# SixLabors/ZlibStream

Measured on AMD Instinct MI355X. Metric: deflate MB/s (input) at level 6, 64 MiB buffers, higher is better.
Workload: dtype u8; 1 GPU; english64: 1 x 67108864-byte pseudo-random-English (Zipf words of alice29.txt) buffer per GPU, level 6, zlib framing, inputs resident in HBM; level=6, buffer_bytes=67108864, buffers_per_gpu=1, compressed_bytes=27425826, parallelism=independent buffers, 1 GPU(s), no collective in the data path

## Files before the change

### zlibstream_amd/csrc/zs_core.h

```cpp
#pragma once
#include <stdint.h>
#include <vector>

#if defined(__HIPCC__)
#include <hip/hip_runtime.h>
#define ZS_HD __host__ __device__ __forceinline__
#define ZS_HD_NOINLINE __host__ __device__
#else
#define ZS_HD inline
#define ZS_HD_NOINLINE
#endif

namespace zs {

constexpr int kMinMatch = 3;
constexpr int kMaxMatch = 258;
constexpr int kMinLookahead = kMaxMatch + kMinMatch + 1;
constexpr int kWSize = 32768;
constexpr int kWMask = kWSize - 1;
constexpr int kWindowSize = 2 * kWSize;
constexpr int kMaxDist = kWSize - kMinLookahead;
constexpr int kSlideAt = kWindowSize - kMinLookahead;
constexpr int kHashBits = 15;
constexpr int kHashSize = 1 << kHashBits;
// ... 479 lines not shown
        uint32_t cK = acc.mK(p), cK4 = acc.mK4(p);
        if (p == 0) cK = cK4 = kNoMatch;
        const Step st = lazy_step(kind, p, pend, cK, cK4, lv);
        if (st.emit) ns++;
        kind = st.kind;
        p = st.pos;
    }
    int node = node_of3(kind, p, cx.cs, ce);
    while (node < kNodeExit3) {
        const uint32_t v = tbl[node];
        ns += node_cnt(v);
        node = node_succ(v);
    }
    return (uint32_t)(node - kNodeExit3) | flags | ((uint32_t)ns << 16);
}

ZS_HD bool slot_valid(const ChunkCtx &cx, int slot, int64_t body_end) {
    if (slot <= 256) return cx.cs + slot <= body_end + 257;
    return cx.cs > 0;
}


ZS_HD int extra_lbits(int code) { return code < 8 ? 0 : (code == 28 ? 0 : (code - 4) >> 2); }
ZS_HD int extra_dbits(int code) { return code < 4 ? 0 : (code - 2) >> 1; }
ZS_HD int extra_blbits(int code) { return code == 16 ? 2 : code == 17 ? 3 : code == 18 ? 7 : 0; }
ZS_HD int base_length(int code) {
    if (code < 8) return code;
    if (code == 28) return 0;
    int e = (code - 4) >> 2;
    return ((4 + (code & 3)) << e);
// ... 507 lines not shown
```

### zlibstream_amd/csrc/zs_device.h

```cpp
#pragma once
#include <cstddef>
#include "zs_core.h"
#include "zs_lit_engine.h"
#include "zs_fast_sweep.h"
#include "zs_rle.h"

namespace zs {

constexpr int kMatchTile = 16384;
constexpr int kMatchBack = 32512;
constexpr int kMatchFwd = 272;
constexpr int kMatchLdsBytes = kMatchBack + kMatchTile + kMatchFwd;
constexpr int kMatchLdsLinks = kMatchBack + kMatchTile;
constexpr int kMatchLds = kMatchLdsBytes + 2 * kMatchLdsLinks;
constexpr int kAdlerPiece = 65536;

constexpr int64_t kScratchWindow = 0;
constexpr int64_t kScratchHead = 66560;
constexpr int64_t kScratchPrev = kScratchHead + 2 * kHashSize;
constexpr int64_t kScratchHead32 = kScratchPrev + 2 * kWSize;
constexpr int64_t kScratchBytes = kScratchHead32 + 4 * kHashSize;

struct StreamDesc {
    const uint8_t *in;
// ... 94 lines not shown
constexpr uint32_t kSpecBail = 1u << 30;
ZS_HD uint32_t spec_pack(int guess, int exit_slot, int count, bool bail) {
    return (uint32_t)guess | ((uint32_t)exit_slot << 9) | ((uint32_t)count << 18) | (bail ? kSpecBail : 0u);
}
ZS_HD int spec_guess(uint32_t r) { return (int)(r & 0x1FF); }
ZS_HD int spec_exit(uint32_t r) { return (int)((r >> 9) & 0x1FF); }
ZS_HD int spec_count(uint32_t r) { return (int)((r >> 18) & 0xFFF); }
constexpr int kSpecMinInput = 1 << 20;
constexpr int kSpecLenBits = 10;
constexpr int kSpecWarm = 128;
constexpr int kSpecRunsDen = 8;
struct K5Spec {
    uint32_t *rec;
    uint32_t *base;
    int len_bits, warm, corrupt;
};
constexpr int kDeferBudget = 8;
constexpr int kCutBudget = 12;

constexpr int kFastChunk = 262144;
constexpr int kFastWarm = 65536;
constexpr int kFastMinInput = 4 << 20;
constexpr int kFastMinPeriodic = 64 << 10;
constexpr int64_t kFastRunSyms = kFastWarm + kFastChunk + 1024;
constexpr int64_t kFastRunBitWords = (kFastWarm + kFastChunk + 2048) / 32;
constexpr int64_t kFastRunScratch = 2 * kHashSize + 4 * kHashSize;
struct FastRunOut {
    int64_t mark_pos, mark_nsyms;
    int64_t end_pos, nsyms;
    int64_t final_base;
    int64_t sym_dst;
// ... 13 lines not shown
```

### zlibstream_amd/csrc/zs_engine.hip

```cpp
#include <hip/hip_runtime.h>

#include <algorithm>
#include <cstdio>
#include <cstdlib>
#include <cstring>
#include <string>
#include <thread>
#include <vector>

#define ZS_BUILDING_LIBRARY
#include "../../include/zsgpu.h"
#include "zs_kernels.hip"
#include "zs_inflate_par.hip"
#include "zs_inflate_tok.hip"
#include "zs_png.hip"
#include "zs_crc32.hip"

using namespace zs;

namespace {

struct DevBuf {
    void *p = nullptr;
    size_t cap = 0;
};

enum Stage {
    kStClear, kStAdler, kStLinks, kStMatch, kStChunkMap, kStSegMap, kStResolve, kStExpand, kStEmitSyms, kStTail, kStTrees,
    kStOffsets, kStEmitBits, kStSpecWalk, kStSpecVerify, kStCrc32, kStCount
};
const char *const kStageNames[kStCount] = {"clear", "adler", "links", "match", "chunkmap", "segmap", "resolve", "expand",
                                           "emit_syms", "tail", "trees", "offsets", "emit_bits", "spec_walk", "spec_verify", "crc32_frame"};

}

struct zs_ctx {
    int device = 0;
    hipStream_t stream = nullptr;
    hipStream_t aux = nullptr;
    hipEvent_t ev_fork = nullptr, ev_join = nullptr, ev_pre0 = nullptr, ev_pre = nullptr;
    hipEvent_t ev_spec[2] = {};
    hipEvent_t ev_part[16] = {};
    std::vector<hipEvent_t> ev_pool;
    std::string err;
    bool profiling = false;
    int fast_fallbacks = 0;
    int round_runs = 0;
    int cut_rounds = 0;
    int lit_fallbacks = 0;
    int spec_streams = 0, spec_fallbacks = 0, spec_wrong_chunks = 0;
    int spec_periodic = 0;
    int64_t dbg_blk_off = 0, dbg_chunk_off = 0, dbg_nchunks = 0, dbg_spec_n = 0, dbg_n_spec = 0;
    int64_t lit_engine_bytes = 0;
    std::vector<int64_t> inf_used;
    int64_t *inf_probe = nullptr;
    int64_t png_segments = 0;
    int fast_rounds = 0;
    bool no_rounds_once = false;
    int last_op = 0;
    hipEvent_t ev[kStCount + 1] = {};
    double stage_ms[kStCount] = {};
    uint32_t *crc_tab = nullptr;
    DevBuf sd, st, work, wpre, geo, link, mm, maps, chunk_far, segmap, supmap, seg_entry, seg_symbase, seg_stale, entry, symbase, stale, syms, blk_end, blk_top, blocks, trees, info, pieces, scratch,
        stage_in, stage_out, wr, inf_desc, inf_state, par_ps, par_st, par_work, par_cbits, par_ccnt, par_surv, par_scnt, par_cands, par_tabs, par_toktabs, par_toks, par_ctoks, par_tokstat, par_tails, par_retry, par_fxtab, par_blocks, par_cells,
        par_windows, par_fail, run_syms, run_bits, run_scratch, run_outs, run_fail, adl_tr, adl_res, plan_blk, ins_bits, mm_bak, cut_pos, cut_bkt, win_groups, win_sg, win_maps, win_entries, persist_bak, resume_flag, rle_tiles, own_in, fr_chunks, fr_meta, fr_planes, fr_prov, fr_base, fr_counters, spec_rec, spec_flags, png_img, png_seg, png_ctr, png_fimg, png_scratch, png_a7img, png_inflated, png_passes, crc_desc, crc_res, png_zs, png_gather;
    uint32_t *crc32_tab = nullptr;
    hipEvent_t ev_crc[2] = {};
    bool resume_poisoned = false;
    void *pinned = nullptr;
    size_t pinned_cap = 0;
    void *pin_io = nullptr;
    size_t pin_io_cap = 0;
    bool pin_io_busy = false;
    void *pin_out = nullptr;
    size_t pin_out_cap = 0;
    bool pin_out_busy = false;
};

namespace {

// ... 419 lines not shown
    size_t n_work = pl.w_clear.size() + pl.w_adler.size() + pl.w_links.size() + pl.w_match.size() + pl.w_chunks.size() +
                    pl.w_segs.size() + pl.w_sups.size() + pl.w_blocks.size() + pl.w_runs.size();
    if (!ensure(c, c->sd, sizeof(StreamDesc) * (size_t)n) || !ensure(c, c->st, sizeof(StreamState) * (size_t)n) ||
        !ensure(c, c->work, sizeof(uint2) * (n_work + 1)) || !ensure(c, c->link, 2 * (size_t)pl.n_pos + 64) ||
        !ensure(c, c->mm, 8 * (size_t)pl.n_pos + 256) ||
        !ensure(c, c->maps, 4 * (size_t)(pl.n_chunks + 1) * kSlots) || !ensure(c, c->segmap, 8 * (size_t)(pl.n_segs + 1) * kSlots) ||
        !ensure(c, c->supmap, 8 * (size_t)(pl.n_sups + 1) * kSlots) || !ensure(c, c->chunk_far, 2 * (size_t)pl.n_chunks + 64) ||
        !ensure(c, c->seg_entry, 2 * (size_t)(pl.n_segs + 2)) || !ensure(c, c->seg_symbase, 4 * (size_t)(pl.n_segs + 2)) ||
        !ensure(c, c->seg_stale, (size_t)pl.n_segs + 64) || !ensure(c, c->entry, 2 * (size_t)(pl.n_chunks + 2)) ||
        !ensure(c, c->symbase, 4 * (size_t)(pl.n_chunks + 2)) || !ensure(c, c->stale, (size_t)pl.n_chunks + 64) ||
        !ensure(c, c->syms, 4 * (size_t)pl.n_syms + 64) || !ensure(c, c->blk_end, 4 * (size_t)pl.n_blocks + 64) ||
        !ensure(c, c->blk_top, 4 * (size_t)pl.n_blocks + 64) || !ensure(c, c->blocks, sizeof(BlockRec) * (size_t)pl.n_blocks) ||
        !ensure(c, c->trees, sizeof(TreeWork) * (size_t)pl.n_blocks) || !ensure(c, c->info, sizeof(BlockInfo) * (size_t)pl.n_blocks) ||
        !ensure(c, c->pieces, 4 * (size_t)pl.n_pieces + 64) || !ensure(c, c->scratch, (size_t)kScratchBytes * (size_t)n) ||
        !ensure(c, c->cut_pos, 8 * (size_t)pl.n_cuts + 64) || !ensure(c, c->cut_bkt, 8 * (size_t)pl.n_cuts + 64) ||
        (pl.n_spec && (!ensure(c, c->spec_rec, 8 * (size_t)pl.n_spec + 64) || !ensure(c, c->spec_flags, 4 * (size_t)n + 64))))
        return false;
    const size_t o_segcl = 16 * (size_t)pl.n_segs, o_cstart = o_segcl + 4 * ((size_t)pl.n_segs + (size_t)n),
                 o_head = o_cstart + 4 * ((size_t)pl.n_chunks + (size_t)n), o_cl = o_head + 4 * (size_t)pl.n_chunks;
    const size_t geo_bytes = o_cl + 4 * pl.cl.size();
    if (!ensure(c, c->geo, geo_bytes + 64)) return false;
    for (int i = 0; i < n; i++) {
        StreamDesc &s = pl.sd[(size_t)i];
        const int32_t *g = (const int32_t *)c->geo.p;
        const uint8_t *gb = (const uint8_t *)c->geo.p;
        s.seg_c0 = g + s.seg_off, s.seg_after = g + pl.n_segs + s.seg_off, s.seg_base = g + 2 * pl.n_segs + s.seg_off;
        s.seg_S = g + 3 * pl.n_segs + s.seg_off;
        s.seg_cl = (const int32_t *)(gb + o_segcl) + s.seg_off + i;
        s.cstart = (const int32_t *)(gb + o_cstart) + s.chunk_off + i;
        s.head = (const int32_t *)(gb + o_head) + s.chunk_off;
        s.cl = (const uint32_t *)(gb + o_cl);
// ... 104 lines not shown
        hipLaunchKernelGGL(zs_zero_kernel, dim3(blocks), dim3(256), 0, stream, z);
        if (ro && ro->resume && pl.sd[0].fv_end >= 0) {
            const int64_t lo = std::max<int64_t>(0, ro->p0 - kWSize - 64) / 32, hi = ro->p0 / 32;
            if (hi > lo) ZS_HIP(c, hipMemsetAsync(pl.sd[0].ins_bits + lo, 0xFF, (size_t)(hi - lo) * 4, stream));
            ZS_HIP(c, hipMemsetD32Async((hipDeviceptr_t)(pl.sd[0].ins_bits + hi), (int)((1u << (ro->p0 & 31)) - 1u), 1, stream));
        }
    }

    const StreamDesc *d_sd = dev<StreamDesc>(c->sd);
    StreamState *d_st = dev<StreamState>(c->st);
    const uint2 *d_work = dev<uint2>(c->work);
    const bool prof = c->profiling;
    const int k5_ahead = getenv("ZS_K5_AHEAD") ? atoi(getenv("ZS_K5_AHEAD")) : 1;
    c->dbg_blk_off = pl.sd[0].blk_off, c->dbg_chunk_off = pl.sd[0].chunk_off, c->dbg_nchunks = pl.sd[0].nchunks;
    c->dbg_spec_n = pl.sd[0].spec_n, c->dbg_n_spec = pl.n_spec;
    const K5Spec k5s{dev<uint32_t>(c->spec_rec), dev<uint32_t>(c->spec_rec) + pl.n_spec, spec_bits, spec_warm, spec_corrupt};
    int spec_ok_streams = 0;
    bool need_maps = true, spec_ran = false;
    if (!rounds) c->spec_streams = c->spec_fallbacks = c->spec_wrong_chunks = c->spec_periodic = 0;
    auto mark = [&](int i) {
        if (prof) (void)hipEventRecord(c->ev[i], stream);
    };
    ht_plan = ht_us();
    ZS_HIP(c, hipEventRecord(c->ev_pre0, stream));
    auto side_work = [&]() -> bool {
        ZS_HIP(c, hipStreamWaitEvent(c->aux, c->ev_pre0, 0));
        if (!pl.w_clear.empty())
            hipLaunchKernelGGL(zs_clear_kernel, dim3((unsigned)pl.w_clear.size()), dim3(256), 0, c->aux, d_sd, d_work + o_clear);
        if (!pl.w_adler.empty())
            hipLaunchKernelGGL(zs_adler_kernel, dim3((unsigned)pl.w_adler.size()), dim3(256), 0, c->aux, d_sd, d_work + o_adler,
                               dev<uint32_t>(c->pieces));
// ... 218 lines not shown
        ZS_HIP(c, hipMemcpyAsync(c->sd.p, c->pinned, sizeof(StreamDesc) * (size_t)n, hipMemcpyHostToDevice, stream));
        if (getenv("ZS_DEBUG")) fprintf(stderr, "zs: %d stream(s) below 4 MiB at level %d: %s\n", n, level, periodic ? "all period, the speculative runs" : "the sweeps");
    }
    mark(3);
    if (strategy == kHuffmanOnly) {
        ZS_HIP(c, hipMemsetAsync(c->mm.p, 0, 8 * (size_t)pl.n_pos + 64, stream));
    } else if (!pl.w_match.empty())
        hipLaunchKernelGGL(zs_match_kernel, dim3((unsigned)pl.w_match.size()), dim3(1024), kMatchLds + 16, stream, d_sd, d_work + o_match,
                           dev<uint16_t>(c->link), dev<uint2>(c->mm), lv, strategy, d_st);
    mark(4);
    if (!side_work()) return false;
    if (pl.n_spec) {
        spec_ran = true;
        hipLaunchKernelGGL((zs_emit_syms_lane_kernel<4, 1>), dim3((unsigned)((pl.max_spec_n + 63) / 64), (unsigned)n), dim3(kK5Threads), 0, stream, d_sd, d_st,
                           (const uint2 *)nullptr, 0, dev<uint2>(c->mm), dev<uint16_t>(c->link), (const uint16_t *)nullptr, (const uint32_t *)nullptr,
                           dev<uint32_t>(c->syms), dev<int32_t>(c->blk_end), dev<int32_t>(c->blk_top), c->crc_tab, lv, strategy, hash_variant, k5_ahead, k5s);
        if (prof) (void)hipEventRecord(c->ev_spec[0], stream);
        hipLaunchKernelGGL(zs_spec_verify_kernel, dim3((unsigned)n), dim3(1024), 0, stream, d_sd, d_st, dev<uint2>(c->mm), dev<uint16_t>(c->link), c->crc_tab, lv,
                           strategy, hash_variant, k5s, dev<int32_t>(c->spec_flags));
        int32_t *hf = (int32_t *)c->pinned;
        ZS_HIP(c, hipMemcpyAsync(hf, c->spec_flags.p, 4 * (size_t)n, hipMemcpyDeviceToHost, stream));
        ZS_HIP(c, hipStreamSynchronize(stream));
        if (prof) (void)hipEventRecord(c->ev_spec[1], stream);
        for (int i = 0; i < n; i++) {
            if (hf[i] == 0) continue;
            c->spec_streams++;
            if (hf[i] == 1) spec_ok_streams++;
            else c->spec_fallbacks++;
            if (hf[i] == 2) c->spec_periodic++;
        }
        if (spec_ok_streams < c->spec_streams) {
// ... 122 lines not shown
                           dev<uint8_t>(c->scratch), c->crc_tab, lv, strategy, hash_variant, level);
        ZS_HIP(c, hipEventRecord(c->ev_join, c->aux));
    }
    if (!pl.w_segs.empty() && need_maps)
        hipLaunchKernelGGL(zs_expand_kernel, dim3((unsigned)((pl.w_segs.size() + 63) / 64)), dim3(64), 0, stream, d_sd, d_st,
                           d_work + o_segs, (int)pl.w_segs.size(), dev<uint2>(c->mm), dev<uint16_t>(c->link),
                           dev<uint32_t>(c->maps), dev<uint16_t>(c->seg_entry), dev<uint32_t>(c->seg_symbase),
                           dev<uint8_t>(c->stale), dev<uint16_t>(c->entry), dev<uint32_t>(c->symbase), c->crc_tab, lv, strategy,
                           hash_variant);
    mark(8);
    if (!pl.w_chunks.empty() && need_maps)
        hipLaunchKernelGGL((zs_emit_syms_lane_kernel<4, 0>), dim3((unsigned)((pl.w_chunks.size() + 63) / 64)), dim3(kK5Threads), 0, stream, d_sd, d_st,
                           d_work + o_chunks, (int)pl.w_chunks.size(), dev<uint2>(c->mm), dev<uint16_t>(c->link), dev<uint16_t>(c->entry),
                           dev<uint32_t>(c->symbase), dev<uint32_t>(c->syms), dev<int32_t>(c->blk_end), dev<int32_t>(c->blk_top),
                           c->crc_tab, lv, strategy, hash_variant, k5_ahead, k5s);
    if (spec_ok_streams)
        hipLaunchKernelGGL((zs_emit_syms_lane_kernel<4, 2>), dim3((unsigned)((pl.max_spec_n + 63) / 64), (unsigned)n), dim3(kK5Threads), 0, stream, d_sd, d_st,
                           (const uint2 *)nullptr, 0, dev<uint2>(c->mm), dev<uint16_t>(c->link), (const uint16_t *)nullptr, (const uint32_t *)nullptr,
                           dev<uint32_t>(c->syms), dev<int32_t>(c->blk_end), dev<int32_t>(c->blk_top), c->crc_tab, lv, strategy, hash_variant, k5_ahead, k5s);
    mark(9);
    if (tail_serial)
        hipLaunchKernelGGL(zs_tail_kernel, dim3((unsigned)n), dim3(1024), kTailLds, stream, d_sd, d_st, dev<uint16_t>(c->link),
                           dev<uint32_t>(c->syms), dev<int32_t>(c->blk_end), dev<int32_t>(c->blk_top), dev<BlockRec>(c->blocks),
                           dev<uint8_t>(c->scratch), c->crc_tab, lv, strategy, hash_variant, level);
    else if (!tail_late) ZS_HIP(c, hipStreamWaitEvent(stream, c->ev_join, 0));
    hipLaunchKernelGGL(zs_body_blocks_kernel, dim3((unsigned)n), dim3(256), 0, stream, d_sd, d_st, dev<int32_t>(c->blk_end),
                       dev<int32_t>(c->blk_top), dev<BlockRec>(c->blocks), dev<uint32_t>(c->syms));
    if (tail_late)
        hipLaunchKernelGGL(zs_tail_kernel, dim3((unsigned)n), dim3(1024), kTailLds, stream, d_sd, d_st, dev<uint16_t>(c->link),
                           dev<uint32_t>(c->syms), dev<int32_t>(c->blk_end), dev<int32_t>(c->blk_top), dev<BlockRec>(c->blocks),
                           dev<uint8_t>(c->scratch), c->crc_tab, lv, strategy, hash_variant, level);
    }
    if (pl.n_runs) {
        if (!getenv("ZS_FAST_NO_PROBE") && force_seq == 0 && !pl.any_dual) {
// ... 104 lines not shown
        for (size_t k = 0; k < nw && k < 24; k++) fprintf(stderr, " %d(end %lld, flush %d)", wb[k], (long long)wr->ends[k], wr->flush.empty() ? 0 : wr->flush[k]);
        fprintf(stderr, "\n");
    }
    if (prof) {
        for (int i = 0; i < kStCount; i++) {
            float ms = 0;
            if (i >= kStLinks && i <= kStEmitBits) (void)hipEventElapsedTime(&ms, c->ev[i], c->ev[i + 1]);
            c->stage_ms[i] = ms;
        }
        if (spec_ran) {
            float a = 0, b = 0, m = 0;
            (void)hipEventElapsedTime(&a, c->ev[kStChunkMap], c->ev_spec[0]);
            (void)hipEventElapsedTime(&b, c->ev_spec[0], c->ev_spec[1]);
            (void)hipEventElapsedTime(&m, c->ev_spec[1], c->ev[kStChunkMap + 1]);
            c->stage_ms[kStSpecWalk] = a, c->stage_ms[kStSpecVerify] = b, c->stage_ms[kStChunkMap] = m;
        }
        if (n_parts) {
            for (int i = kStLinks; i <= kStTail; i++) c->stage_ms[i] = 0;
            for (const TimedPair &t : pairs) {
                float ms = 0;
                (void)hipEventElapsedTime(&ms, t.a, t.b);
                c->stage_ms[t.stage] += ms;
            }
        }
    }
    {
        bool any_poison = false;
        std::vector<uint8_t> fl(force_lit ? *force_lit : std::vector<uint8_t>((size_t)n, 0));
        for (int i = 0; i < n; i++)
            if (hst[i].poison) any_poison = true, fl[(size_t)i] = 1;
// ... 184 lines not shown
    if (hipFuncGetAttributes(&fa, (const void *)zs_match_kernel) != hipSuccess || fa.sharedSizeBytes != 0) {
        fprintf(stderr, "zsgpu: zs_match_kernel has static LDS; its tile addressing assumes none\n");
        zs_ctx_destroy(c);
        return ZS_STREAM_ERROR;
    }
    *out = c;
    return ZS_OK;
}

void zs_ctx_destroy(zs_ctx *c) {
    if (!c) return;
    (void)hipSetDevice(c->device);
    DevBuf *bufs[] = {&c->sd, &c->st, &c->work, &c->wpre, &c->geo, &c->link, &c->mm, &c->maps, &c->chunk_far, &c->segmap, &c->supmap, &c->seg_entry, &c->seg_symbase, &c->seg_stale, &c->entry, &c->symbase, &c->stale, &c->syms,
                      &c->blk_end, &c->blk_top, &c->blocks, &c->trees, &c->info, &c->pieces, &c->scratch, &c->stage_in, &c->stage_out, &c->wr, &c->inf_desc, &c->inf_state, &c->par_ps, &c->par_st, &c->par_work, &c->par_cbits, &c->par_ccnt, &c->par_surv, &c->par_scnt,
                      &c->par_cands, &c->par_tabs, &c->par_toktabs, &c->par_toks, &c->par_ctoks, &c->par_tokstat, &c->par_tails, &c->par_retry, &c->par_fxtab, &c->par_blocks, &c->par_cells, &c->par_windows, &c->par_fail, &c->run_syms, &c->run_bits,
                      &c->run_scratch, &c->run_outs, &c->run_fail, &c->adl_tr, &c->adl_res, &c->plan_blk, &c->ins_bits, &c->mm_bak, &c->cut_pos, &c->cut_bkt, &c->win_groups, &c->win_sg, &c->win_maps, &c->win_entries, &c->persist_bak, &c->resume_flag, &c->rle_tiles, &c->own_in, &c->fr_chunks, &c->fr_meta, &c->fr_planes, &c->fr_prov, &c->fr_base, &c->fr_counters, &c->spec_rec, &c->spec_flags, &c->png_img, &c->png_seg, &c->png_ctr, &c->png_fimg, &c->png_scratch, &c->png_a7img, &c->png_inflated, &c->png_passes, &c->crc_desc, &c->crc_res, &c->png_zs, &c->png_gather};
    for (DevBuf *b : bufs)
        if (b->p) (void)hipFree(b->p);
    if (c->crc_tab) (void)hipFree(c->crc_tab);
    if (c->crc32_tab) (void)hipFree(c->crc32_tab);
    for (auto &e : c->ev_crc)
        if (e) (void)hipEventDestroy(e);
    if (c->pinned) (void)hipHostFree(c->pinned);
    if (c->pin_io) (void)hipHostFree(c->pin_io);
    if (c->pin_out) (void)hipHostFree(c->pin_out);
    for (auto &e : c->ev)
        if (e) (void)hipEventDestroy(e);
    for (auto &e : c->ev_part)
        if (e) (void)hipEventDestroy(e);
    for (auto &e : c->ev_spec)
        if (e) (void)hipEventDestroy(e);
// ... 47 lines not shown
        memcpy(out, state, sizeof state);
        return sizeof state;
    }
    if (k == "blk_end") src = dev<int32_t>(c->blk_end) + c->dbg_blk_off, bytes = 4 * (int64_t)(ss.body_syms / kBlockSyms);
    else if (k == "blk_top") src = dev<int32_t>(c->blk_top) + c->dbg_blk_off, bytes = 4 * (int64_t)(ss.body_syms / kBlockSyms);
    else if (k == "symbase") src = dev<uint32_t>(c->symbase) + c->dbg_chunk_off, bytes = 4 * c->dbg_nchunks;
    else if (k == "spec_base") src = dev<uint32_t>(c->spec_rec) + c->dbg_n_spec, bytes = 4 * c->dbg_spec_n;
    else return -1;
    if (bytes > cap || (bytes > 0 && !src)) return -1;
    if (bytes > 0 && hipMemcpy(out, src, (size_t)bytes, hipMemcpyDeviceToHost) != hipSuccess) return -1;
    return bytes;
}

const char *zs_ctx_stage_name(const zs_ctx *c, int s) {
    static const char *const inf_names[6] = {"inf_find", "inf_measure", "inf_chain", "inf_decode", "inf_windows", "inf_resolve"};
    if (s == kStCrc32) return kStageNames[s];
    if (c && c->last_op == 1) return s >= 0 && s < 6 ? inf_names[s] : "";
    if (c && c->last_op == 2 && s == kStExpand) return "fast_sweep";
    if (c && c->last_op == 2 && s == kStTail) return "fast_runs+tail";
    return s >= 0 && s < kStCount ? kStageNames[s] : "";
}
double zs_ctx_stage_ms(const zs_ctx *c, int s) { return c && s >= 0 && s < kStCount ? c->stage_ms[s] : 0.0; }

int zs_deflate_batch_device(zs_ctx *c, int n, const void *const *in, const int64_t *in_len, void *const *out,
                            const int64_t *out_cap, int64_t *out_len, int *status, int level, int strategy, int hash_variant,
                            void *hip_stream) {
    if (!check_args(c, n, in_len, level, strategy)) return ZS_STREAM_ERROR;
    if (n == 0) return ZS_OK;
    if (hipSetDevice(c->device) != hipSuccess) return ZS_STREAM_ERROR;
    hipStream_t s = hip_stream ? (hipStream_t)hip_stream : c->stream;
    int rc = ZS_OK;
// ... 1511 lines not shown
```

### zlibstream_amd/csrc/zs_kernels.hip

```cpp
#include <hip/hip_runtime.h>

#include <type_traits>

#include "zs_device.h"
#include "zs_png.h"

namespace zs {

typedef uint32_t __attribute__((aligned(1))) u32u;
typedef uint64_t __attribute__((aligned(1))) u64u;
typedef const __attribute__((address_space(1))) uint8_t *gcbytes;
typedef __attribute__((address_space(1))) uint8_t *gbytes_w;
__device__ __forceinline__ gcbytes as_global(const uint8_t *p) { return (gcbytes)(uintptr_t)p; }
__device__ __forceinline__ gbytes_w as_global(uint8_t *p) { return (gbytes_w)(uintptr_t)p; }
typedef const __attribute__((address_space(1))) uint32_t __attribute__((aligned(1))) *gcu32u;
typedef const __attribute__((address_space(1))) uint64_t __attribute__((aligned(1))) *gcu64u;
__device__ __forceinline__ uint32_t g_u32_bytes(gcbytes p) {
    return (uint32_t)p[0] | ((uint32_t)p[1] << 8) | ((uint32_t)p[2] << 16) | ((uint32_t)p[3] << 24);
}
typedef uint32_t u32x4 __attribute__((ext_vector_type(4)));
typedef const __attribute__((address_space(1))) u32x4 *gcu32x4;
__device__ __forceinline__ uint32_t lds_u32(const uint8_t *base, int idx) {
    const uint32_t *q = (const uint32_t *)(base + (idx & ~3));
    return __builtin_amdgcn_alignbyte(q[1], q[0], (uint32_t)idx & 3u);
// ... 1690 lines not shown
    }
    struct Done {
        lds_u32p slot;
        __device__ ~Done() { k5_publish(slot, kK5Done); }
    } done{sh_line};
    const int i = blockIdx.x * 64 + lane;
    int si, c;
    if constexpr (MODE == 0) {
        if (i >= nwork) return;
        const uint2 w = work[i];
        if (st[w.x].deferred || st[w.x].spec_ok) return;
        si = (int)w.x, c = (int)w.y;
    } else {
        si = (int)blockIdx.y, c = i;
        if (!sd[si].spec || c >= sd[si].spec_n) return;
        if (MODE == 1 ? spec_periodic(sd[si], st[si]) : !st[si].spec_ok) return;
    }
    const StreamDesc s = sd[si];
    GlobalAcc acc{as_global(s.in), mm + s.pos_off, crc_tab_g, strategy, hash_variant, link + s.pos_off};
    const uint32_t base = MODE == 0 ? symbase[s.chunk_off + c] : MODE == 2 ? sp.base[s.spec_off + c] : 0u;
    GlobalSymSink sink(syms + s.sym_off + base, base, blk_end + s.blk_off, blk_top + s.blk_off);
    int kind, ns;
    int64_t p;
    uint32_t pflags = 0;
    NullEv nev;
    const ChunkCtx cx = MODE == 0 ? chunk_ctx(s, c) : spec_chunk_ctx(s, c, sp.len_bits);
    if constexpr (MODE == 1) {
        kind = kR, ns = 0, p = cx.cs - sp.warm;
        p = (c == 0 || p < 0) ? 0 : p;
    } else {
        chunk_special_prefix(acc, sink, cx, MODE == 0 ? (int)entry[s.chunk_off + c] : spec_guess(sp.rec[s.spec_off + c]), lv, strategy, kind, p, ns,
                             pflags, nev);
    }
    const int64_t ce = cx.ce;
    if (MODE != 1 && p >= ce) return;
    const uint2 *a = acc.mm;
    const gcbytes gin = acc.in;
    uint32_t pend = kNoMatch;
    if (kind == kXK) pend = acc.mK(p - 1);
    else if (kind == kXK4) pend = acc.mK4(p - 1);
    uint8_t lit = p >= 1 ? gin[p - 1] : 0;
    const bool rec_lits = strategy != kHuffmanOnly;
    uint2 cur = a[p];
    if (p == 0) cur.x &= ~kRecMask, cur.y = 0;
    static_assert(kNoMatch == 0 && kMinMatch == 3, "record arithmetic below");
    const uint32_t klm = strategy == kFiltered ? 2u : 0u, kdm = strategy == kFiltered ? 0u : (uint32_t)kTooFar;
    const int q_last = s.n - 1, lazy = lv.lazy, good = lv.good;
    int q = (int)p;
    const int64_t gi0 = s.pos_off + q;
    const int q0 = q - (int)(gi0 & 15);
    const uint32_t ring_lane = (uint32_t)(uintptr_t)(__attribute__((address_space(3))) uint8_t *)sh_ring_ + (uint32_t)lane * 128u;
    k5_publish(sh_base, (uint32_t)(gi0 >> 4));
    k5_publish(sh_last, (uint32_t)(q_last - q0) >> 4);
    auto steps = [&](auto rl_tag, auto ring_tag, const int q_end) {
        constexpr bool kRecLits = decltype(rl_tag)::value, kRing = decltype(ring_tag)::value;
        uint32_t dsym = 0;
        int dns = -1, dend = 0, dtop = 0;
#ifdef ZS_FV_PROF
        long long k5t0 = wall_clock64();
        int k5steps = 0, k5miss = 0, k5lanemiss = 0, k5mysteps = 0;
#endif
        while (q < q_end) {
            if constexpr (MODE != 1)
                if (dns >= 0) sink(dns, dsym, dend, dtop);
            const int m = pend ? (int)(pend >> 16) + 3 : 2;
            int qa = q + 1, qb = q - 1 + m;
            qa = qa > q_last ? q_last : qa;
            qb = qb > q_last ? q_last : qb;
            qb = pend ? qb : qa;
            uint2 na, nb;
            int32_t filled = 0;
            if constexpr (kRing) {
                const uint32_t ua = (uint32_t)(qa - q0), ub = (uint32_t)(qb - q0);
                k5_publish(sh_line, (uint32_t)(q - q0) >> 4);
                filled = (int32_t)k5_peek(sh_filled);
                const uint64_t ra = k5_peek64(ring_lane + (k5_slot<kK5Ring>(ua >> 4) << 13) + ((ua & 15u) << 3));
                const uint64_t rb = k5_peek64(ring_lane + (k5_slot<kK5Ring>(ub >> 4) << 13) + ((ub & 15u) << 3));
                na = make_uint2((uint32_t)ra, (uint32_t)(ra >> 32));
                nb = make_uint2((uint32_t)rb, (uint32_t)(rb >> 32));
// ... 29 lines not shown
                k5miss += __ballot((int32_t)((uint32_t)(qn - q0) >> 4) > filled) != 0;
                k5lanemiss += (int32_t)((uint32_t)(qn - q0) >> 4) > filled;
#endif
                if ((int32_t)((uint32_t)(qn - q0) >> 4) > filled) {
                    uint64_t rec;
                    asm volatile("global_load_dwordx2 %0, %1, off\n\ts_waitcnt vmcnt(0)" : "=&v"(rec) : "v"(a + qn) : "memory");
                    cur = make_uint2((uint32_t)rec, (uint32_t)(rec >> 32));
                }
            } else {
                cur = npos == q + 1 ? na : nb;
            }
            asm volatile("" ::"v"(cur.x), "v"(cur.y));
            lit = nlit;
            q = npos;
        }
        if constexpr (MODE != 1)
            if (dns >= 0) sink(dns, dsym, dend, dtop);
#ifdef ZS_FV_PROF
        if (kRing && (blockIdx.x & 63) == 7 && (lane == 0 || lane == 37))
            printf("K5PROF block %d lane %d: my steps %d, my misses %d; steps with a miss in the wave %d; ticks (100 MHz) %lld\n", (int)blockIdx.x, lane,
                   k5mysteps, k5lanemiss, k5miss, wall_clock64() - k5t0);
#endif
    };
    auto run_to = [&](const int q_end) {
        if (!rec_lits) steps(std::false_type{}, std::false_type{}, q_end);
        else if (ahead > 0) steps(std::true_type{}, std::true_type{}, q_end);
        else steps(std::true_type{}, std::false_type{}, q_end);
    };
    if constexpr (MODE != 1) {
        run_to((int)ce);
    } else {
        const int cs = (int)cx.cs;
        run_to(cs);
        const int guess = kind == kR ? q - cs : 256 + kind;
        ns = 0;
        if (cx.m != 0) {
            NullSink nsk;
            chunk_special_prefix(acc, nsk, cx, guess, lv, strategy, kind, p, ns, pflags, nev);
            q = (int)p;
            pend = kind == kXK ? acc.mK(p - 1) : kind == kXK4 ? acc.mK4(p - 1) : kNoMatch;
            lit = gin[p - 1];
            cur = a[p];
        }
        run_to((int)ce);
        const int exit_slot = kind == kR ? q - (int)ce : 256 + kind;
        const int told = c == sp.corrupt ? (guess + 1) % kSlots : guess;
        sp.rec[s.spec_off + c] = spec_pack(told, exit_slot, ns, (pflags & (kMapEqualBit | kMapPoisonBit)) != 0);
    }
}

__global__ __launch_bounds__(1024) void zs_spec_verify_kernel(const StreamDesc *sd, StreamState *st, const uint2 *mm, const uint16_t *link,
                                                             const uint32_t *crc_tab_g, LevelCfg lv, int strategy, int hash_variant, K5Spec sp,
                                                             int32_t *flags) {
    constexpr int kTile = 8192, kPer = kTile / 1024;
    __shared__ uint32_t sh_rec[kTile];
    __shared__ uint32_t sh_wave[16];
    __shared__ int sh_bad, sh_wrong;
    __shared__ uint32_t sh_carry, sh_prev;
    const int si = (int)blockIdx.x, t = (int)threadIdx.x;
// ... 83 lines not shown
        NullSink nsk;
        int k2, n2;
        int64_t p2;
        uint32_t f2;
        chunk_special_prefix(acc, nsk, cx, g, lv, strategy, k2, p2, n2, f2, lev);
        k_done = k;
        preins = lev.pos >= 0 ? lev.pos + 1 : -1;
        break;
    }
    ss.k_done = k_done;
    ss.preins = (int32_t)preins;
    ss.body_syms = sh_carry;
    ss.deferred = 0;
    ss.spec_ok = 1, ss.spec_wrong = 0;
    flags[si] = 1;
}

__global__ __launch_bounds__(256) void zs_body_blocks_kernel(const StreamDesc *sd, const StreamState *st, const int32_t *blk_end,
                                                             const int32_t *blk_top, BlockRec *blocks, uint32_t *syms) {
    const StreamDesc s = sd[blockIdx.x];
    if (s.fast_runs > 0 || st[blockIdx.x].deferred) return;
    if (s.resume)
        for (uint32_t i = threadIdx.x; i < s.start_syms; i += blockDim.x) syms[s.sym_off + i] = s.persist->syms[i];
    const int nb_body = (int)(st[blockIdx.x].body_syms / kBlockSyms);
    BlockRec *blk = blocks + s.blk_off;
    for (int i = threadIdx.x; i < nb_body; i += blockDim.x) {
        int64_t start = i ? blk_end[s.blk_off + i - 1] : (s.resume ? s.start_block : 0);
        int64_t end = blk_end[s.blk_off + i];
        BlockRec r;
        r.start = start;
// ... 1374 lines not shown
```

Before: 14650 MB/s.

## Store speculative walk symbols in slabs and compact instead of re-walking

The speculative walk kernel now writes each chunk's symbols into a per-chunk slab buffer, including an 'odd' marker from the special prefix. After verification, a new compact kernel copies the slabs into the final symbol array and reconstructs block-end and block-top entries with a wave reduction of symbol lengths. This replaces the second full lane-walk pass (MODE 2) that recomputed the symbols. In exchange it adds slab memory traffic and allocation, and makes the walk write symbols even for chunks whose guess may later prove wrong.

```diff
diff --git a/zlibstream_amd/csrc/zs_core.h b/zlibstream_amd/csrc/zs_core.h
--- a/zlibstream_amd/csrc/zs_core.h
+++ b/zlibstream_amd/csrc/zs_core.h
@@ -517,6 +517,26 @@
     }
     return (uint32_t)(node - kNodeExit3) | flags | ((uint32_t)ns << 16);
 }
+
+constexpr int kSpecSlabPad = 32;
+constexpr int kSpecMaxLenBits = 11;
+ZS_HD constexpr int spec_slab_stride(int len_bits) { return (1 << len_bits) + kSpecSlabPad; }
+ZS_HD int sym_len(uint32_t sym) { return (sym >> 16) ? (int)(sym & 0xFFFFu) + kMinMatch : 1; }
+ZS_HD int spec_cut_index(uint32_t base, int count) {
+    const uint32_t i = (base / (uint32_t)kBlockSyms + 1u) * (uint32_t)kBlockSyms - 1u - base;
+    return i < (uint32_t)count ? (int)i : -1;
+}
+ZS_HD int64_t spec_first_start(int64_t cs, int slot) { return slot <= 256 ? cs + slot : cs - 1; }
+ZS_HD int64_t spec_sym_end(int64_t start, uint32_t sym) { return start + sym_len(sym); }
+ZS_HD int64_t spec_sym_top(int64_t start, bool odd) { return start + (odd ? 2 : 1); }
+struct SpecSlabSink {
+    uint32_t *out;
+    int odd;
+    ZS_HD void operator()(int i, uint32_t sym, int64_t end, int64_t top) {
+        out[i] = sym;
+        if (top != spec_sym_top(end - sym_len(sym), false)) odd = i;
+    }
+};
 
 ZS_HD bool slot_valid(const ChunkCtx &cx, int slot, int64_t body_end) {
     if (slot <= 256) return cx.cs + slot <= body_end + 257;
diff --git a/zlibstream_amd/csrc/zs_device.h b/zlibstream_amd/csrc/zs_device.h
--- a/zlibstream_amd/csrc/zs_device.h
+++ b/zlibstream_amd/csrc/zs_device.h
@@ -132,7 +132,10 @@
     uint32_t *rec;
     uint32_t *base;
     int len_bits, warm, corrupt;
+    uint32_t *syms;
+    int stride;
 };
+static_assert(spec_slab_stride(kSpecMaxLenBits) - kSpecSlabPad <= 0xFFF, "spec_pack's count field holds the symbols of the longest chunk");
 constexpr int kDeferBudget = 8;
 constexpr int kCutBudget = 12;
 
diff --git a/zlibstream_amd/csrc/zs_engine.hip b/zlibstream_amd/csrc/zs_engine.hip
--- a/zlibstream_amd/csrc/zs_engine.hip
+++ b/zlibstream_amd/csrc/zs_engine.hip
@@ -27,10 +27,11 @@
 
 enum Stage {
     kStClear, kStAdler, kStLinks, kStMatch, kStChunkMap, kStSegMap, kStResolve, kStExpand, kStEmitSyms, kStTail, kStTrees,
-    kStOffsets, kStEmitBits, kStSpecWalk, kStSpecVerify, kStCrc32, kStCount
+    kStOffsets, kStEmitBits, kStSpecWalk, kStSpecVerify, kStCrc32, kStSpecCompact, kStCount
 };
 const char *const kStageNames[kStCount] = {"clear", "adler", "links", "match", "chunkmap", "segmap", "resolve", "expand",
-                                           "emit_syms", "tail", "trees", "offsets", "emit_bits", "spec_walk", "spec_verify", "crc32_frame"};
+                                           "emit_syms", "tail", "trees", "offsets", "emit_bits", "spec_walk", "spec_verify", "crc32_frame",
+                                           "spec_compact"};
 
 }
 
@@ -39,7 +40,7 @@
     hipStream_t stream = nullptr;
     hipStream_t aux = nullptr;
     hipEvent_t ev_fork = nullptr, ev_join = nullptr, ev_pre0 = nullptr, ev_pre = nullptr;
-    hipEvent_t ev_spec[2] = {};
+    hipEvent_t ev_spec[4] = {};
     hipEvent_t ev_part[16] = {};
     std::vector<hipEvent_t> ev_pool;
     std::string err;
@@ -63,7 +64,7 @@
     uint32_t *crc_tab = nullptr;
     DevBuf sd, st, work, wpre, geo, link, mm, maps, chunk_far, segmap, supmap, seg_entry, seg_symbase, seg_stale, entry, symbase, stale, syms, blk_end, blk_top, blocks, trees, info, pieces, scratch,
         stage_in, stage_out, wr, inf_desc, inf_state, par_ps, par_st, par_work, par_cbits, par_ccnt, par_surv, par_scnt, par_cands, par_tabs, par_toktabs, par_toks, par_ctoks, par_tokstat, par_tails, par_retry, par_fxtab, par_blocks, par_cells,
-        par_windows, par_fail, run_syms, run_bits, run_scratch, run_outs, run_fail, adl_tr, adl_res, plan_blk, ins_bits, mm_bak, cut_pos, cut_bkt, win_groups, win_sg, win_maps, win_entries, persist_bak, resume_flag, rle_tiles, own_in, fr_chunks, fr_meta, fr_planes, fr_prov, fr_base, fr_counters, spec_rec, spec_flags, png_img, png_seg, png_ctr, png_fimg, png_scratch, png_a7img, png_inflated, png_passes, crc_desc, crc_res, png_zs, png_gather;
+        par_windows, par_fail, run_syms, run_bits, run_scratch, run_outs, run_fail, adl_tr, adl_res, plan_blk, ins_bits, mm_bak, cut_pos, cut_bkt, win_groups, win_sg, win_maps, win_entries, persist_bak, resume_flag, rle_tiles, own_in, fr_chunks, fr_meta, fr_planes, fr_prov, fr_base, fr_counters, spec_rec, spec_flags, spec_syms, png_img, png_seg, png_ctr, png_fimg, png_scratch, png_a7img, png_inflated, png_passes, crc_desc, crc_res, png_zs, png_gather;
     uint32_t *crc32_tab = nullptr;
     hipEvent_t ev_crc[2] = {};
     bool resume_poisoned = false;
@@ -513,7 +514,8 @@
         !ensure(c, c->trees, sizeof(TreeWork) * (size_t)pl.n_blocks) || !ensure(c, c->info, sizeof(BlockInfo) * (size_t)pl.n_blocks) ||
         !ensure(c, c->pieces, 4 * (size_t)pl.n_pieces + 64) || !ensure(c, c->scratch, (size_t)kScratchBytes * (size_t)n) ||
         !ensure(c, c->cut_pos, 8 * (size_t)pl.n_cuts + 64) || !ensure(c, c->cut_bkt, 8 * (size_t)pl.n_cuts + 64) ||
-        (pl.n_spec && (!ensure(c, c->spec_rec, 8 * (size_t)pl.n_spec + 64) || !ensure(c, c->spec_flags, 4 * (size_t)n + 64))))
+        (pl.n_spec && (!ensure(c, c->spec_rec, 8 * (size_t)pl.n_spec + 64) || !ensure(c, c->spec_flags, 4 * (size_t)n + 64) ||
+                       !ensure(c, c->spec_syms, 4 * (size_t)pl.n_spec * (size_t)spec_slab_stride(spec_bits) + 64))))
         return false;
     const size_t o_segcl = 16 * (size_t)pl.n_segs, o_cstart = o_segcl + 4 * ((size_t)pl.n_segs + (size_t)n),
                  o_head = o_cstart + 4 * ((size_t)pl.n_chunks + (size_t)n), o_cl = o_head + 4 * (size_t)pl.n_chunks;
@@ -648,7 +650,8 @@
     const int k5_ahead = getenv("ZS_K5_AHEAD") ? atoi(getenv("ZS_K5_AHEAD")) : 1;
     c->dbg_blk_off = pl.sd[0].blk_off, c->dbg_chunk_off = pl.sd[0].chunk_off, c->dbg_nchunks = pl.sd[0].nchunks;
     c->dbg_spec_n = pl.sd[0].spec_n, c->dbg_n_spec = pl.n_spec;
-    const K5Spec k5s{dev<uint32_t>(c->spec_rec), dev<uint32_t>(c->spec_rec) + pl.n_spec, spec_bits, spec_warm, spec_corrupt};
+    const K5Spec k5s{dev<uint32_t>(c->spec_rec), dev<uint32_t>(c->spec_rec) + pl.n_spec, spec_bits, spec_warm, spec_corrupt,
+                     dev<uint32_t>(c->spec_syms), spec_slab_stride(spec_bits)};
     int spec_ok_streams = 0;
     bool need_maps = true, spec_ran = false;
     if (!rounds) c->spec_streams = c->spec_fallbacks = c->spec_wrong_chunks = c->spec_periodic = 0;
@@ -897,7 +900,7 @@
         spec_ran = true;
         hipLaunchKernelGGL((zs_emit_syms_lane_kernel<4, 1>), dim3((unsigned)((pl.max_spec_n + 63) / 64), (unsigned)n), dim3(kK5Threads), 0, stream, d_sd, d_st,
                            (const uint2 *)nullptr, 0, dev<uint2>(c->mm), dev<uint16_t>(c->link), (const uint16_t *)nullptr, (const uint32_t *)nullptr,
-                           dev<uint32_t>(c->syms), dev<int32_t>(c->blk_end), dev<int32_t>(c->blk_top), c->crc_tab, lv, strategy, hash_variant, k5_ahead, k5s);
+                           (uint32_t *)nullptr, (int32_t *)nullptr, (int32_t *)nullptr, c->crc_tab, lv, strategy, hash_variant, k5_ahead, k5s);
         if (prof) (void)hipEventRecord(c->ev_spec[0], stream);
         hipLaunchKernelGGL(zs_spec_verify_kernel, dim3((unsigned)n), dim3(1024), 0, stream, d_sd, d_st, dev<uint2>(c->mm), dev<uint16_t>(c->link), c->crc_tab, lv,
                            strategy, hash_variant, k5s, dev<int32_t>(c->spec_flags));
@@ -1050,10 +1053,12 @@
                            d_work + o_chunks, (int)pl.w_chunks.size(), dev<uint2>(c->mm), dev<uint16_t>(c->link), dev<uint16_t>(c->entry),
                            dev<uint32_t>(c->symbase), dev<uint32_t>(c->syms), dev<int32_t>(c->blk_end), dev<int32_t>(c->blk_top),
                            c->crc_tab, lv, strategy, hash_variant, k5_ahead, k5s);
-    if (spec_ok_streams)
-        hipLaunchKernelGGL((zs_emit_syms_lane_kernel<4, 2>), dim3((unsigned)((pl.max_spec_n + 63) / 64), (unsigned)n), dim3(kK5Threads), 0, stream, d_sd, d_st,
-                           (const uint2 *)nullptr, 0, dev<uint2>(c->mm), dev<uint16_t>(c->link), (const uint16_t *)nullptr, (const uint32_t *)nullptr,
-                           dev<uint32_t>(c->syms), dev<int32_t>(c->blk_end), dev<int32_t>(c->blk_top), c->crc_tab, lv, strategy, hash_variant, k5_ahead, k5s);
+    if (spec_ok_streams) {
+        if (prof) (void)hipEventRecord(c->ev_spec[2], stream);
+        hipLaunchKernelGGL(zs_spec_compact_kernel, dim3((unsigned)((pl.max_spec_n + 3) / 4), (unsigned)n), dim3(256), 0, stream, d_sd, d_st, k5s,
+                           dev<uint32_t>(c->syms), dev<int32_t>(c->blk_end), dev<int32_t>(c->blk_top));
+        if (prof) (void)hipEventRecord(c->ev_spec[3], stream);
+    }
     mark(9);
     if (tail_serial)
         hipLaunchKernelGGL(zs_tail_kernel, dim3((unsigned)n), dim3(1024), kTailLds, stream, d_sd, d_st, dev<uint16_t>(c->link),
@@ -1188,6 +1193,9 @@
             (void)hipEventElapsedTime(&b, c->ev_spec[0], c->ev_spec[1]);
             (void)hipEventElapsedTime(&m, c->ev_spec[1], c->ev[kStChunkMap + 1]);
             c->stage_ms[kStSpecWalk] = a, c->stage_ms[kStSpecVerify] = b, c->stage_ms[kStChunkMap] = m;
+            float k = 0;
+            if (spec_ok_streams) (void)hipEventElapsedTime(&k, c->ev_spec[2], c->ev_spec[3]);
+            c->stage_ms[kStSpecCompact] = k;
         }
         if (n_parts) {
             for (int i = kStLinks; i <= kStTail; i++) c->stage_ms[i] = 0;
@@ -1402,7 +1410,7 @@
     DevBuf *bufs[] = {&c->sd, &c->st, &c->work, &c->wpre, &c->geo, &c->link, &c->mm, &c->maps, &c->chunk_far, &c->segmap, &c->supmap, &c->seg_entry, &c->seg_symbase, &c->seg_stale, &c->entry, &c->symbase, &c->stale, &c->syms,
                       &c->blk_end, &c->blk_top, &c->blocks, &c->trees, &c->info, &c->pieces, &c->scratch, &c->stage_in, &c->stage_out, &c->wr, &c->inf_desc, &c->inf_state, &c->par_ps, &c->par_st, &c->par_work, &c->par_cbits, &c->par_ccnt, &c->par_surv, &c->par_scnt,
                       &c->par_cands, &c->par_tabs, &c->par_toktabs, &c->par_toks, &c->par_ctoks, &c->par_tokstat, &c->par_tails, &c->par_retry, &c->par_fxtab, &c->par_blocks, &c->par_cells, &c->par_windows, &c->par_fail, &c->run_syms, &c->run_bits,
-                      &c->run_scratch, &c->run_outs, &c->run_fail, &c->adl_tr, &c->adl_res, &c->plan_blk, &c->ins_bits, &c->mm_bak, &c->cut_pos, &c->cut_bkt, &c->win_groups, &c->win_sg, &c->win_maps, &c->win_entries, &c->persist_bak, &c->resume_flag, &c->rle_tiles, &c->own_in, &c->fr_chunks, &c->fr_meta, &c->fr_planes, &c->fr_prov, &c->fr_base, &c->fr_counters, &c->spec_rec, &c->spec_flags, &c->png_img, &c->png_seg, &c->png_ctr, &c->png_fimg, &c->png_scratch, &c->png_a7img, &c->png_inflated, &c->png_passes, &c->crc_desc, &c->crc_res, &c->png_zs, &c->png_gather};
+                      &c->run_scratch, &c->run_outs, &c->run_fail, &c->adl_tr, &c->adl_res, &c->plan_blk, &c->ins_bits, &c->mm_bak, &c->cut_pos, &c->cut_bkt, &c->win_groups, &c->win_sg, &c->win_maps, &c->win_entries, &c->persist_bak, &c->resume_flag, &c->rle_tiles, &c->own_in, &c->fr_chunks, &c->fr_meta, &c->fr_planes, &c->fr_prov, &c->fr_base, &c->fr_counters, &c->spec_rec, &c->spec_flags, &c->spec_syms, &c->png_img, &c->png_seg, &c->png_ctr, &c->png_fimg, &c->png_scratch, &c->png_a7img, &c->png_inflated, &c->png_passes, &c->crc_desc, &c->crc_res, &c->png_zs, &c->png_gather};
     for (DevBuf *b : bufs)
         if (b->p) (void)hipFree(b->p);
     if (c->crc_tab) (void)hipFree(c->crc_tab);
@@ -1480,7 +1488,7 @@
 
 const char *zs_ctx_stage_name(const zs_ctx *c, int s) {
     static const char *const inf_names[6] = {"inf_find", "inf_measure", "inf_chain", "inf_decode", "inf_windows", "inf_resolve"};
-    if (s == kStCrc32) return kStageNames[s];
+    if (s == kStCrc32 || s == kStSpecCompact) return kStageNames[s];
     if (c && c->last_op == 1) return s >= 0 && s < 6 ? inf_names[s] : "";
     if (c && c->last_op == 2 && s == kStExpand) return "fast_sweep";
     if (c && c->last_op == 2 && s == kStTail) return "fast_runs+tail";
diff --git a/zlibstream_amd/csrc/zs_kernels.hip b/zlibstream_amd/csrc/zs_kernels.hip
--- a/zlibstream_amd/csrc/zs_kernels.hip
+++ b/zlibstream_amd/csrc/zs_kernels.hip
@@ -1728,12 +1728,14 @@
     } else {
         si = (int)blockIdx.y, c = i;
         if (!sd[si].spec || c >= sd[si].spec_n) return;
-        if (MODE == 1 ? spec_periodic(sd[si], st[si]) : !st[si].spec_ok) return;
+        if (spec_periodic(sd[si], st[si])) return;
     }
     const StreamDesc s = sd[si];
     GlobalAcc acc{as_global(s.in), mm + s.pos_off, crc_tab_g, strategy, hash_variant, link + s.pos_off};
-    const uint32_t base = MODE == 0 ? symbase[s.chunk_off + c] : MODE == 2 ? sp.base[s.spec_off + c] : 0u;
-    GlobalSymSink sink(syms + s.sym_off + base, base, blk_end + s.blk_off, blk_top + s.blk_off);
+    const uint32_t base = MODE == 0 ? symbase[s.chunk_off + c] : 0u;
+    GlobalSymSink sink(MODE == 0 ? syms + s.sym_off + base : nullptr, base, MODE == 0 ? blk_end + s.blk_off : nullptr,
+                       MODE == 0 ? blk_top + s.blk_off : nullptr);
+    uint32_t *const slab = MODE == 1 ? sp.syms + (size_t)(s.spec_off + c) * (size_t)sp.stride : nullptr;
     int kind, ns;
     int64_t p;
     uint32_t pflags = 0;
@@ -1743,8 +1745,7 @@
         kind = kR, ns = 0, p = cx.cs - sp.warm;
         p = (c == 0 || p < 0) ? 0 : p;
     } else {
-        chunk_special_prefix(acc, sink, cx, MODE == 0 ? (int)entry[s.chunk_off + c] : spec_guess(sp.rec[s.spec_off + c]), lv, strategy, kind, p, ns,
-                             pflags, nev);
+        chunk_special_prefix(acc, sink, cx, (int)entry[s.chunk_off + c], lv, strategy, kind, p, ns, pflags, nev);
     }
     const int64_t ce = cx.ce;
     if (MODE != 1 && p >= ce) return;
@@ -1766,8 +1767,8 @@
     const uint32_t ring_lane = (uint32_t)(uintptr_t)(__attribute__((address_space(3))) uint8_t *)sh_ring_ + (uint32_t)lane * 128u;
     k5_publish(sh_base, (uint32_t)(gi0 >> 4));
     k5_publish(sh_last, (uint32_t)(q_last - q0) >> 4);
-    auto steps = [&](auto rl_tag, auto ring_tag, const int q_end) {
-        constexpr bool kRecLits = decltype(rl_tag)::value, kRing = decltype(ring_tag)::value;
+    auto steps = [&](auto rl_tag, auto ring_tag, auto emit_tag, const int q_end) {
+        constexpr bool kRecLits = decltype(rl_tag)::value, kRing = decltype(ring_tag)::value, kEmit = decltype(emit_tag)::value;
         uint32_t dsym = 0;
         int dns = -1, dend = 0, dtop = 0;
 #ifdef ZS_FV_PROF
@@ -1775,8 +1776,11 @@
         int k5steps = 0, k5miss = 0, k5lanemiss = 0, k5mysteps = 0;
 #endif
         while (q < q_end) {
-            if constexpr (MODE != 1)
-                if (dns >= 0) sink(dns, dsym, dend, dtop);
+            if constexpr (kEmit)
+                if (dns >= 0) {
+                    if constexpr (MODE == 0) sink(dns, dsym, dend, dtop);
+                    else slab[dns] = dsym;
+                }
             const int m = pend ? (int)(pend >> 16) + 3 : 2;
             int qa = q + 1, qb = q - 1 + m;
             qa = qa > q_last ? q_last : qa;
@@ -1836,35 +1840,39 @@
             lit = nlit;
             q = npos;
         }
-        if constexpr (MODE != 1)
-            if (dns >= 0) sink(dns, dsym, dend, dtop);
+        if constexpr (kEmit)
+            if (dns >= 0) {
+                if constexpr (MODE == 0) sink(dns, dsym, dend, dtop);
+                else slab[dns] = dsym;
+            }
 #ifdef ZS_FV_PROF
         if (kRing && (blockIdx.x & 63) == 7 && (lane == 0 || lane == 37))
             printf("K5PROF block %d lane %d: my steps %d, my misses %d; steps with a miss in the wave %d; ticks (100 MHz) %lld\n", (int)blockIdx.x, lane,
                    k5mysteps, k5lanemiss, k5miss, wall_clock64() - k5t0);
 #endif
     };
-    auto run_to = [&](const int q_end) {
-        if (!rec_lits) steps(std::false_type{}, std::false_type{}, q_end);
-        else if (ahead > 0) steps(std::true_type{}, std::true_type{}, q_end);
-        else steps(std::true_type{}, std::false_type{}, q_end);
+    auto run_to = [&](auto emit_tag, const int q_end) {
+        if (!rec_lits) steps(std::false_type{}, std::false_type{}, emit_tag, q_end);
+        else if (ahead > 0) steps(std::true_type{}, std::true_type{}, emit_tag, q_end);
+        else steps(std::true_type{}, std::false_type{}, emit_tag, q_end);
     };
     if constexpr (MODE != 1) {
-        run_to((int)ce);
+        run_to(std::true_type{}, (int)ce);
     } else {
         const int cs = (int)cx.cs;
-        run_to(cs);
+        run_to(std::false_type{}, cs);
         const int guess = kind == kR ? q - cs : 256 + kind;
         ns = 0;
         if (cx.m != 0) {
-            NullSink nsk;
-            chunk_special_prefix(acc, nsk, cx, guess, lv, strategy, kind, p, ns, pflags, nev);
+            SpecSlabSink ssk{slab, -1};
+            chunk_special_prefix(acc, ssk, cx, guess, lv, strategy, kind, p, ns, pflags, nev);
+            slab[sp.stride - 1] = (uint32_t)ssk.odd;
             q = (int)p;
             pend = kind == kXK ? acc.mK(p - 1) : kind == kXK4 ? acc.mK4(p - 1) : kNoMatch;
             lit = gin[p - 1];
             cur = a[p];
         }
-        run_to((int)ce);
+        run_to(std::true_type{}, (int)ce);
         const int exit_slot = kind == kR ? q - (int)ce : 256 + kind;
         const int told = c == sp.corrupt ? (guess + 1) % kSlots : guess;
         sp.rec[s.spec_off + c] = spec_pack(told, exit_slot, ns, (pflags & (kMapEqualBit | kMapPoisonBit)) != 0);
@@ -1978,6 +1986,33 @@
     ss.deferred = 0;
     ss.spec_ok = 1, ss.spec_wrong = 0;
     flags[si] = 1;
+}
+
+__global__ __launch_bounds__(256) void zs_spec_compact_kernel(const StreamDesc *sd, const StreamState *st, K5Spec sp, uint32_t *syms, int32_t *blk_end,
+                                                             int32_t *blk_top) {
+    const int si = (int)blockIdx.y, c = (int)blockIdx.x * 4 + (int)(threadIdx.x >> 6), lane = (int)(threadIdx.x & 63);
+    const StreamDesc &s = sd[si];
+    if (!s.spec || c >= s.spec_n || !st[si].spec_ok) return;
+    const uint32_t r = sp.rec[s.spec_off + c], base = sp.base[s.spec_off + c];
+    const int count = spec_count(r), cut = spec_cut_index(base, count);
+    const uint32_t *slab = sp.syms + (size_t)(s.spec_off + c) * (size_t)sp.stride;
+    uint32_t *out = syms + s.sym_off + base;
+    int before = 0;
+    for (int i = lane; i < count; i += 64) {
+        const uint32_t v = slab[i];
+        out[i] = v;
+        before += i < cut ? sym_len(v) : 0;
+    }
+    if (cut < 0) return;
+#pragma unroll
+    for (int d = 32; d >= 1; d >>= 1) before += __shfl_xor(before, d, 64);
+    if (lane != 0) return;
+    const ChunkCtx cx = spec_chunk_ctx(s, c, sp.len_bits);
+    const int64_t start = spec_first_start(cx.cs, spec_guess(r)) + before;
+    const bool odd = cx.m != 0 && slab[sp.stride - 1] == (uint32_t)cut;
+    const uint32_t bi = (base + (uint32_t)cut) / kBlockSyms;
+    blk_end[s.blk_off + bi] = (int32_t)spec_sym_end(start, slab[cut]);
+    blk_top[s.blk_off + bi] = (int32_t)spec_sym_top(start, odd);
 }
 
 __global__ __launch_bounds__(256) void zs_body_blocks_kernel(const StreamDesc *sd, const StreamState *st, const int32_t *blk_end,
```

New measurement: 15190 MB/s (median of 6 runs). 3.7% higher.
